# zouyuoz/SVS-UNet-PyTorch

Hardware: AMD Instinct MI355X
Metric: spectrogram-tiles/sec (512x128) U-Net fwd+bwd (L1 train step incl. Adam) (higher is better)
Workload: dtype f32; 1 GPU; train.py L1-loss step, 512x128 tiles, batch 64 per GPU; global_batch=64, parallelism=dp1, mode=train

## Files before the change

### svs_unet_pytorch_amd/csrc/gemm_wgrad.hip

```cpp
#include <stdlib.h>

#include "gemm_pipeline.h"
#include "internal.h"
#include "mfma_split.h"

struct WgradArgs {
  const float* s; long lds; int Hs, Ws, Cs;
  const float* l; long ldl; int Hl, Wl, Cl;
  int B;
  float* slab;
  long pix_per_split;
  int ws_shift, hs_shift;
  int b_shift;
};

template <int T> __device__ __forceinline__ void load_vec(const float* p, float (&f)[T]);
template <> __device__ __forceinline__ void load_vec<4>(const float* p, float (&f)[4]) {
  const f32x4 v = *(const f32x4*)p; f[0] = v[0]; f[1] = v[1]; f[2] = v[2]; f[3] = v[3];
}
template <> __device__ __forceinline__ void load_vec<2>(const float* p, float (&f)[2]) {
  const float2 v = *(const float2*)p; f[0] = v.x; f[1] = v.y;
}
template <int T> __device__ __forceinline__ void store_vec(float* p, const float (&f)[T]);
template <> __device__ __forceinline__ void store_vec<4>(float* p, const float (&f)[4]) { *(f32x4*)p = (f32x4){f[0], f[1], f[2], f[3]}; }
// ... 162 lines not shown

  auto multiply = [&](int buf) __attribute__((always_inline)) {
    if constexpr (SPLIT) {
      float ga[4][TM], gb[4][TN];
#pragma unroll
      for (int k = 0; k < 4; ++k) {
        const int kr = 4 * q + k;
        load_vec<TM>(&As[buf][kr * LDA + wm * (TM * 16) + TM * lrow], ga[k]);
        load_vec<TN>(&Bs[buf][kr * LDB + wn * (TN * 16) + TN * lrow], gb[k]);
      }
      SvsSplitA sa[TM];
      SvsSplitB sb[TN];
#pragma unroll
      for (int i = 0; i < TM; ++i) sa[i] = svs_split_a(ga[0][i], ga[1][i], ga[2][i], ga[3][i]);
#pragma unroll
      for (int j = 0; j < TN; ++j) sb[j] = svs_split_b(gb[0][j], gb[1][j], gb[2][j], gb[3][j]);
      svs_mma_split<TM, TN>(acc, sa, sb);
    } else {
#pragma unroll
    for (int k = 0; k < 4; ++k) {
      float fa[TM], fb[TN];
      const int kr = 4 * q + k;
      load_vec<TM>(&As[buf][kr * LDA + wm * (TM * 16) + TM * lrow], fa);
      load_vec<TN>(&Bs[buf][kr * LDB + wn * (TN * 16) + TN * lrow], fb);
#pragma unroll
      for (int i = 0; i < TM; ++i)
#pragma unroll
        for (int j = 0; j < TN; ++j)
          acc[i][j] = __builtin_amdgcn_mfma_f32_16x16x4f32(fa[i], fb[j], acc[i][j], 0, 0, 0);
    }
    }
  };
  auto fetch = [&](int pk, auto setc) __attribute__((always_inline)) {
    constexpr int set_ = decltype(setc)::value;
    if (SKIP) load_tile_skip(pk, ra[set_], rb[set_]);
    else load_tile(pk, ra[set_], rb[set_]);
  };
  svs_k_loop<PF>(first_valid((int)p_begin), (int)p_end, [&](int pk) { return first_valid(pk + 16); }, fetch, store_tile, multiply);

  float* slab = p.slab + (long)blockIdx.z * p.Cs * Ntot;
#pragma unroll
  for (int i = 0; i < TM; ++i)
#pragma unroll
    for (int r = 0; r < 4; ++r) {
      const int cs = cs0 + wm * (TM * 16) + TM * (4 * q + r) + i;
      const int n = n0 + wn * (TN * 16) + TN * lrow;
      if (n < Ntot) {
        float v[TN];
#pragma unroll
        for (int j = 0; j < TN; ++j) v[j] = acc[i][j][r];
        store_vec<TN>(&slab[(long)cs * Ntot + n], v);
      }
    }
}

struct WgWinArgs {
  const float* s; long lds; const float* l; long ldl;
  int B, Hs, Ws, Cs, Hl, Wl, Cl;
  float* slab;
  int ntiles, tiles_per_block;
};

template <int MT>
__global__ __launch_bounds__(256, 2) void wgrad_window_kernel(WgWinArgs p) {
  constexpr int TH = 4, TW = 16, KS = 4 / MT, CSB = 16 * MT;
  constexpr int LS = CSB + 16;
  constexpr int LH = 2 * TH + 3, LW = 2 * TW + 3, LL = 24;
  constexpr int NS = TH * TW * (CSB / 4), NL = LH * LW * 4;
  constexpr int RS = (NS + 255) / 256, RL = (NL + 255) / 256;
  constexpr int KSTEPS = TH * TW / 4 / KS;
  constexpr unsigned OOB = 0x80000000u;
  __shared__ __attribute__((aligned(16))) float Ssm[TH * TW * LS];
  __shared__ __attribute__((aligned(16))) float Lsm[LH * LW * LL];
  const int t = threadIdx.x, lane = t & 63, wave = t >> 6;
  const int lrow = lane & 15, q = lane >> 4;
  const int mt = wave % MT, half = wave / MT;
  const int mchunks = p.Cs / CSB;
  const int m0 = (blockIdx.y % mchunks) * CSB, cl0 = (blockIdx.y / mchunks) * 16;
  const int tiles_w = (p.Ws + TW - 1) / TW, tiles_h = (p.Hs + TH - 1) / TH;
  const int tile_lo = blockIdx.x * p.tiles_per_block;
  const int tile_hi = min(tile_lo + p.tiles_per_block, p.ntiles);

  f32x4 sreg[RS], lreg[RL];
  auto fetch = [&](int tile) {
    const int tw0 = (tile % tiles_w) * TW, th0 = ((tile / tiles_w) % tiles_h) * TH;
    const long b = tile / (tiles_w * tiles_h);
    const __amdgpu_buffer_rsrc_t rs = __builtin_amdgcn_make_buffer_rsrc((void*)(p.s + b * p.Hs * p.Ws * p.lds), 0, OOB, 0x00020000);
    const __amdgpu_buffer_rsrc_t rl = __builtin_amdgcn_make_buffer_rsrc((void*)(p.l + b * p.Hl * p.Wl * p.ldl), 0, OOB, 0x00020000);
#pragma unroll
    for (int r = 0; r < RS; ++r) {
      const int e = t + 256 * r;
      const int c4 = e % (CSB / 4), px = e / (CSB / 4);
      const int sh = th0 + px / TW, sw = tw0 + px % TW;
      const bool ok = e < NS && sh < p.Hs && sw < p.Ws;
      const unsigned vo = ok ? (unsigned)(((sh * p.Ws + sw) * (int)p.lds + m0 + c4 * 4) * 4) : OOB;
      sreg[r] = __builtin_bit_cast(f32x4, __builtin_amdgcn_raw_buffer_load_b128(rs, (int)vo, 0, 0));
    }
#pragma unroll
    for (int r = 0; r < RL; ++r) {
      const int e = t + 256 * r;
      const int c4 = e & 3, px = e >> 2;
      const int ih = 2 * th0 - 2 + px / LW, iw = 2 * tw0 - 2 + px % LW;
      const bool ok = e < NL && (unsigned)ih < (unsigned)p.Hl && (unsigned)iw < (unsigned)p.Wl;
      const unsigned vo = ok ? (unsigned)(((ih * p.Wl + iw) * (int)p.ldl + cl0 + c4 * 4) * 4) : OOB;
      lreg[r] = __builtin_bit_cast(f32x4, __builtin_amdgcn_raw_buffer_load_b128(rl, (int)vo, 0, 0));
    }
  };
  auto stage = [&]() {
#pragma unroll
    for (int r = 0; r < RS; ++r) {
      const int e = t + 256 * r;
      if (e < NS) *(f32x4*)(&Ssm[(e / (CSB / 4)) * LS + (e % (CSB / 4)) * 4]) = sreg[r];
    }
#pragma unroll
    for (int r = 0; r < RL; ++r) {
      const int e = t + 256 * r;
      if (e < NL) *(f32x4*)(&Lsm[(e >> 2) * LL + (e & 3) * 4]) = lreg[r];
    }
  };

  f32x4 acc[25];
#pragma unroll
  for (int i = 0; i < 25; ++i) acc[i] = (f32x4){0.f, 0.f, 0.f, 0.f};
  const float* abase = &Ssm[(half * (TH / KS) * TW + q) * LS + mt * 16 + lrow];
  const float* bbase = &Lsm[(half * (TH / KS) * 2 * LW + 2 * q) * LL + lrow];

  if (tile_lo < tile_hi) fetch(tile_lo);
  for (int tile = tile_lo; tile < tile_hi; ++tile) {
    __syncthreads();
    stage();
    __syncthreads();
    if (tile + 1 < tile_hi) fetch(tile + 1);
#pragma unroll
    for (int ks = 0; ks < KSTEPS; ++ks) {
      const int sh = ks / 4, sg = ks % 4;
      const float a = abase[(sh * TW + sg * 4) * LS];
#pragma unroll
      for (int tap = 0; tap < 25; ++tap) {
        const int kh = tap / 5, kw = tap % 5;
        const float bv = bbase[((2 * sh + kh) * LW + 8 * sg + kw) * LL];
        acc[tap] = __builtin_amdgcn_mfma_f32_16x16x4f32(a, bv, acc[tap], 0, 0, 0);
      }
    }
  }
  const int Ntot = 25 * p.Cl;
  float* slab = p.slab + ((long)blockIdx.x * KS + half) * p.Cs * Ntot;
#pragma unroll
  for (int tap = 0; tap < 25; ++tap)
#pragma unroll
    for (int r = 0; r < 4; ++r)
      slab[(long)(m0 + mt * 16 + 4 * q + r) * Ntot + tap * p.Cl + cl0 + lrow] = acc[tap][r];
}

__global__ __launch_bounds__(256) void wgrad_reduce_kernel(const float* __restrict__ slab, int ksplit, int Cs, int Cl,
                                                           float* __restrict__ dw) {
  __shared__ float tile[25][65];
  const int clt = Cl < 64 ? Cl : 64;
  const int cs = blockIdx.x, cl0 = blockIdx.y * clt;
  const long zstride = (long)Cs * Cl * 25;
  const float* src0 = slab + (long)cs * 25 * Cl + cl0;
  const int q4 = clt >> 2;
  for (int e = threadIdx.x; e < 25 * q4; e += 256) {
    const int tap = e / q4, cl = (e - tap * q4) * 4;
    const float* src = src0 + (long)tap * Cl + cl;
    f32x4 acc = {0.f, 0.f, 0.f, 0.f};
    int z = 0;
    for (; z + 4 <= ksplit; z += 4, src += 4 * zstride) {
      const f32x4 a = *(const f32x4*)src, b = *(const f32x4*)(src + zstride), c = *(const f32x4*)(src + 2 * zstride), d = *(const f32x4*)(src + 3 * zstride);
      acc += a; acc += b; acc += c; acc += d;
    }
    for (; z < ksplit; ++z, src += zstride) acc += *(const f32x4*)src;
    tile[tap][cl] = acc[0]; tile[tap][cl + 1] = acc[1]; tile[tap][cl + 2] = acc[2]; tile[tap][cl + 3] = acc[3];
  }
  __syncthreads();
  float* dst = dw + ((long)cs * Cl + cl0) * 25;
  for (int e = threadIdx.x; e < 25 * clt; e += 256) {
    const int cl = e / 25, tap = e - cl * 25;
    dst[e] = tile[tap][cl];
  }
}

struct WgradTile { int cfg, BM, BN, ksplit; long pps; };
static WgradTile plan_wgrad(int B, int Hs, int Ws, int Cs, int Cl) {
  WgradTile pl{};
  if (Cs % 128 == 0) { pl.cfg = 0; pl.BM = 128; }
  else if (Cs % 64 == 0) { pl.cfg = 1; pl.BM = 64; }
  else { pl.cfg = 2; pl.BM = 32; }
  if (pl.cfg == 0 && ((long)B * Hs * Ws <= 1024 || Cl <= 32)) { pl.cfg = 1; pl.BM = 64; }
  if (svs_tune_on(SVS_TUNE_WGRAD_CFG)) {
    const int c = (int)svs_tune(SVS_TUNE_WGRAD_CFG);
    if (c == 0 && Cs % 128 == 0) { pl.cfg = 0; pl.BM = 128; }
    if (c == 1 && Cs % 64 == 0) { pl.cfg = 1; pl.BM = 64; }
    if (c == 2 && Cs % 32 == 0) { pl.cfg = 2; pl.BM = 32; }
  }
  pl.BN = 128;
  const long P = (long)B * Hs * Ws;
  const long blocks_mn = (long)(Cs / pl.BM) * ((25L * Cl + pl.BN - 1) / pl.BN);
  long ks = (1024 + blocks_mn - 1) / blocks_mn;
  const long cap = P / 128 > 1 ? P / 128 : 1;
  if (ks > cap) ks = cap;
  if (ks > 512) ks = 512;
  if (ks < 1) ks = 1;
  if (svs_tune_on(SVS_TUNE_WGRAD_KSPLIT)) { long f = svs_tune(SVS_TUNE_WGRAD_KSPLIT); if (f >= 1 && f <= cap) ks = f; }
  long pps = (P + ks - 1) / ks;
  pps = (pps + 15) / 16 * 16;
  ks = (P + pps - 1) / pps;
  pl.ksplit = (int)ks;
  pl.pps = pps;
  return pl;
}

#define WG_GROUPS 8

struct WgWinPlan { int eligible, use, MT, gy, gx, tpb, ntiles, nslab; };
static WgWinPlan plan_wgrad_window(int B, int Hs, int Ws, int Cs, int Cl) {
  WgWinPlan w{};
  w.eligible = (Cl == 16 || Cl == 32) && (Cs == 32 || Cs == 64 || Cs == 128);
  w.ntiles = B * ((Hs + 3) / 4) * ((Ws + 15) / 16);
  w.use = w.eligible && w.ntiles >= 1024;
  if (svs_tune_on(SVS_TUNE_WGRAD_WINDOW)) { const int f = (int)svs_tune(SVS_TUNE_WGRAD_WINDOW); w.use = (f == 0) ? 0 : (f == 2) ? w.eligible : w.use; }
  if (!w.eligible) return w;
  w.MT = (Cs % 64 == 0) ? 4 : 2;
  w.gy = (Cs / (16 * w.MT)) * (Cl / 16);
  int gx = 512 / w.gy;
  if (gx > w.ntiles) gx = w.ntiles;
  w.tpb = (w.ntiles + gx - 1) / gx;
  w.gx = (w.ntiles + w.tpb - 1) / w.tpb;
  w.nslab = w.gx * (4 / w.MT);
  return w;
}

static constexpr int wgrad_gemm_pf(int BM, bool skip) { return skip && BM != 32 ? 2 : 1; }

struct WgradPlan {
  WgWinPlan win;
  WgradTile tile;
  int WM, WN;
  bool skip, split;
  dim3 grid;
  int nslab;
};
static WgradPlan plan_wgrad_call(int B, int Hs, int Ws, int Cs, int Cl, long lds, int Hl, int Wl, long ldl) {
  WgradPlan p{};
  p.win = plan_wgrad_window(B, Hs, Ws, Cs, Cl);
  p.win.use = p.win.use && (long)Hs * Ws * lds * 4 < (1L << 31) && (long)Hl * Wl * ldl * 4 < (1L << 31);
  if (p.win.use) {
    p.grid = dim3(p.win.gx, p.win.gy);
    p.nslab = p.win.nslab;
    return p;
  }
  p.tile = plan_wgrad(B, Hs, Ws, Cs, Cl);
  p.WM = p.tile.cfg == 0 ? 2 : 1;
  p.WN = 4 / p.WM;
  const bool can_skip = B >= 16 && (B & (B - 1)) == 0 && (Ws & (Ws - 1)) == 0 && (long)B * Hs * Ws * lds * 4 < (1L << 31);
  const long f = svs_tune(SVS_TUNE_WGRAD_SKIP);
  p.skip = f == 0 ? false : f == 2 ? can_skip : can_skip && Ws <= 8;
  p.split = svs_tune(SVS_TUNE_MFMA_SPLIT) > 0;
  p.grid = dim3((unsigned)(Cs / p.tile.BM), (unsigned)((25 * Cl + p.tile.BN - 1) / p.tile.BN), (unsigned)p.tile.ksplit);
  p.nslab = p.tile.ksplit;
  return p;
}

size_t svs_wgrad_gemm_workspace(int B, int Hs, int Ws, int Cs, int Cl) {
  const WgWinPlan w = plan_wgrad_window(B, Hs, Ws, Cs, Cl);
  int nslab = plan_wgrad(B, Hs, Ws, Cs, Cl).ksplit;
  if (w.eligible && w.nslab > nslab) nslab = w.nslab;
  return ((size_t)nslab + WG_GROUPS) * Cs * 25 * Cl * sizeof(float);
}

static int wgrad_reduce_run(const float* slabs, int nslab, int Cs, int Cl, float* dw, float* tmp, hipStream_t stream) {
  const long n = (long)Cs * 25 * Cl;
  if (nslab > 2 * WG_GROUPS) {
    const int per = (nslab + WG_GROUPS - 1) / WG_GROUPS;
    const int groups = (nslab + per - 1) / per;
    if (int rc = svs_reduce_slabs_run(slabs, nslab, per, groups, n, tmp, stream)) return rc;
    slabs = tmp;
    nslab = groups;
  }
  hipLaunchKernelGGL(wgrad_reduce_kernel, dim3((unsigned)Cs, (unsigned)((Cl + 63) / 64)), dim3(256), 0, stream, slabs, nslab, Cs,
                     Cl, dw);
  SVS_CHECK_LAUNCH("wgrad_reduce");
  return SVS_OK;
}

template <bool SPLIT, int BM, int WM, int WN>
static void launch_wgrad_tile(const WgradArgs& a, const WgradPlan& p, hipStream_t stream) {
  if (p.skip) hipLaunchKernelGGL((wgrad_gemm_kernel<BM, 128, WM, WN, true, SPLIT, wgrad_gemm_pf(BM, true)>), p.grid, dim3(256), 0, stream, a);
  else hipLaunchKernelGGL((wgrad_gemm_kernel<BM, 128, WM, WN, false, SPLIT, wgrad_gemm_pf(BM, false)>), p.grid, dim3(256), 0, stream, a);
}
template <bool SPLIT>
static void launch_wgrad_gemm(const WgradArgs& a, const WgradPlan& p, hipStream_t stream) {
  switch (p.tile.cfg) {
    case 0: launch_wgrad_tile<SPLIT, 128, 2, 2>(a, p, stream); break;
    case 1: launch_wgrad_tile<SPLIT, 64, 1, 4>(a, p, stream); break;
    default: launch_wgrad_tile<SPLIT, 32, 1, 4>(a, p, stream); break;
  }
}

int svs_wgrad_gemm_run(const float* s, long lds, int B, int Hs, int Ws, int Cs, const float* l, long ldl, int Hl,
                       int Wl, int Cl, float* dw, void* ws, size_t ws_bytes, hipStream_t stream, const char* who) {
  SVS_REQUIRE(s && l && dw, "%s: null pointer", who);
  SVS_REQUIRE(Cs >= 32 && Cs % 32 == 0 && Cl >= 16 && Cl % 4 == 0, "%s: unsupported channels Cs=%d Cl=%d", who, Cs, Cl);
  SVS_REQUIRE(Hs == svs_conv_out(Hl) && Ws == svs_conv_out(Wl), "%s: small grid %dx%d does not match %dx%d", who, Hs, Ws, Hl, Wl);
  SVS_REQUIRE(lds >= Cs && lds % 4 == 0 && ldl >= Cl && ldl % 4 == 0, "%s: bad ld", who);
  SVS_REQUIRE(svs_aligned16(s) && svs_aligned16(l) && svs_aligned16(ws), "%s: pointers must be 16-byte aligned", who);
  const size_t need = svs_wgrad_gemm_workspace(B, Hs, Ws, Cs, Cl);
  if (!ws || ws_bytes < need) {
    svs_set_error("%s: workspace too small (%zu < %zu)", who, ws_bytes, need);
    return SVS_ERR_WORKSPACE;
  }
  const WgradPlan p = plan_wgrad_call(B, Hs, Ws, Cs, Cl, lds, Hl, Wl, ldl);
  if (p.win.use) {
    WgWinArgs wa{s, lds, l, ldl, B, Hs, Ws, Cs, Hl, Wl, Cl, (float*)ws, p.win.ntiles, p.win.tpb};
    if (p.win.MT == 4) hipLaunchKernelGGL((wgrad_window_kernel<4>), p.grid, dim3(256), 0, stream, wa);
    else hipLaunchKernelGGL((wgrad_window_kernel<2>), p.grid, dim3(256), 0, stream, wa);
    SVS_CHECK_LAUNCH("wgrad_window");
  } else {
    WgradArgs a{};
    a.s = s; a.lds = lds; a.Hs = Hs; a.Ws = Ws; a.Cs = Cs;
    a.l = l; a.ldl = ldl; a.Hl = Hl; a.Wl = Wl; a.Cl = Cl;
    a.B = B; a.slab = (float*)ws; a.pix_per_split = p.tile.pps;
    auto log2_or_neg = [](int v) { int s = 0; while ((1 << s) < v) ++s; return (1 << s) == v ? s : -1; };
    a.ws_shift = log2_or_neg(Ws); a.hs_shift = log2_or_neg(Hs);
    SVS_REQUIRE((long)B * Hs * Ws < (1L << 31), "%s: pixel count exceeds 2^31", who);
    SVS_REQUIRE((long)B * Hl * Wl * ldl * 4 < (1L << 31) && (long)(p.tile.pps + 16) * lds * 4 < (1L << 31),
                "%s: operand views need 64-bit offsets; split the batch", who);
    if (p.skip) a.b_shift = log2_or_neg(B);
    if (p.split) launch_wgrad_gemm<true>(a, p, stream);
    else launch_wgrad_gemm<false>(a, p, stream);
    SVS_CHECK_LAUNCH("wgrad_gemm");
  }
  if (svs_tune_flag(SVS_TUNE_SKIP_REDUCE)) return SVS_OK;
  return wgrad_reduce_run((const float*)ws, p.nslab, Cs, Cl, dw, (float*)ws + (size_t)p.nslab * Cs * 25 * Cl, stream);
}

int svs_wgrad_gemm_describe(int B, int Hs, int Ws, int Cs, int Cl, char* buf, size_t n) {
  const WgradPlan p = plan_wgrad_call(B, Hs, Ws, Cs, Cl, Cs, 2 * Hs, 2 * Ws, Cl);
  if (p.win.use) snprintf(buf, n, "wgrad_window_kernel<%d>", p.win.MT);
  else snprintf(buf, n, "wgrad_gemm_kernel<%d, %d, %d, %d, %s, %s, %d>", p.tile.BM, p.tile.BN, p.WM, p.WN, p.skip ? "true" : "false",
                p.split ? "true" : "false", wgrad_gemm_pf(p.tile.BM, p.skip));
  return p.nslab;
}
```

### svs_unet_pytorch_amd/csrc/internal.h

```cpp
#pragma once
#include "common.h"

enum { SVS_MODE_GATHER = 0, SVS_MODE_PARITY = 1 };

int svs_conv_gemm_run(int mode, const float* x, long ldx, int B, int H, int W, int C, const float* wp,
                      const float* bias, const float* scale, const float* shift, float slope, float* y, long ldy,
                      int Ho, int Wo, int N, int accumulate, void* ws, size_t ws_bytes, hipStream_t stream,
                      const char* who, float* stats = nullptr, int stats_cap = 0, int* stats_nblk = nullptr);
int svs_bn_finalize_run(const void* partial, int nblk, long P, int C, float eps, float momentum, float* running_mean,
                        float* running_var, long long* nbt, float* save_mean, float* save_invstd, hipStream_t stream);
int svs_bn_fin_act_apply_run(const void* partial, int rows, const float* raw, long ldr, long P, int C, long pixels_per_sample,
                             const float* gamma, const float* beta, float eps, float momentum, float* running_mean,
                             float* running_var, long long* nbt, float* save_mean, float* save_invstd, float slope,
                             const float* drop, float* y, long ldy, hipStream_t stream);
struct SvsSumJobs { int njobs; const float* partial[12]; int nblk[12]; int C[12]; float* out[12]; };
int svs_channel_sum_finalize_multi_run(const SvsSumJobs& jobs, hipStream_t stream);
size_t svs_bn_partial_floats(long P, int C);
int svs_bn_partial_rows(long P, int C);
size_t svs_conv_gemm_workspace(int mode, int B, int H, int W, int C, int Ho, int Wo, int N);

int svs_wgrad_gemm_run(const float* s, long lds, int B, int Hs, int Ws, int Cs, const float* l, long ldl, int Hl,
                       int Wl, int Cl, float* dw, void* ws, size_t ws_bytes, hipStream_t stream, const char* who);
size_t svs_wgrad_gemm_workspace(int B, int Hs, int Ws, int Cs, int Cl);

int svs_conv_c1_run(const float* x, int B, int H, int W, const float* w, const float* bias, const float* scale,
                    const float* shift, float slope, float* y, long ldy, int N, int accumulate, hipStream_t stream,
                    const char* who, long half = 0);
int svs_deconv_to1_run(const float* x, long ldx, int B, int H, int W, int C, const float* w, const float* bias,
                       float* y, int Ho, int Wo, int apply_sigmoid, hipStream_t stream, const char* who, long half = 0);
int svs_wgrad_c1_run(const float* s, long lds, int B, int Hs, int Ws, int Cs, const float* l, int Hl, int Wl,
                     float* dw, void* ws, size_t ws_bytes, hipStream_t stream, const char* who, long half = 0);
size_t svs_wgrad_c1_workspace(int B, int Hs, int Ws, int Cs);

int svs_channel_sum_run(const float* x, long ldx, long P, int C, float* out, void* ws, size_t ws_bytes, hipStream_t stream);
int svs_sum_run(const float* x, long n, float* out, void* ws, size_t ws_bytes, hipStream_t stream);
int svs_sigmoid_bwd_run(const float* mask, const float* dmask, long n, float* d_logit, hipStream_t stream);

int svs_reduce_slabs_run(const float* slab, int nslab, int per, int groups, long n, float* out, hipStream_t stream);

struct SvsPackJob { const float* w; float* wp; int N, C, kind, first_block; };
struct SvsPackJobs { SvsPackJob j[20]; int n; };
int svs_pack_all_run(SvsPackJobs& jobs, hipStream_t stream);

int svs_bn_bwd_run(const float* dy, long lddy, const float* raw, long ldr, long P, int C, long pixels_per_sample,
                   const float* gamma, const float* beta, const float* save_mean, const float* save_invstd, float slope,
                   const float* drop, float* d_raw, float* dgamma, float* dbeta, float* dbias, void* ws, size_t ws_bytes,
                   hipStream_t stream, float* dbias_partial = nullptr, SvsSumJobs* defer = nullptr);

int svs_fft_twiddles(int n, hipStream_t stream, const float2** out);
int svs_fft_hann(int n, hipStream_t stream, const float** out);

int svs_conv_gemm_describe(int mode, int B, int H, int W, int C, int Ho, int Wo, int N, long ldx, char* buf, size_t n);
int svs_wgrad_gemm_describe(int B, int Hs, int Ws, int Cs, int Cl, char* buf, size_t n);
int svs_conv_bf16_describe(int mode, int B, int H, int W, int C, int Ho, int Wo, int N, char* buf, size_t n);
```

### svs_unet_pytorch_amd/csrc/special.hip

```cpp
#include "internal.h"

struct C1Args {
  const float* x; int B, H, W;
  const float* w;
  const float* bias; const float* scale; const float* shift; float slope;
  float* y; long ldy; int Ho, Wo; int accumulate;
  long half;
};

__device__ __forceinline__ long chan_off(long pix, long ld, int sub, int subs_per_half, long half) {
  return pix * ld + (half ? (sub >= subs_per_half ? half + (sub - subs_per_half) * 4 : sub * 4) : sub * 4);
}

template <int COUT>
__global__ __launch_bounds__(256) void conv_c1_kernel(C1Args p) {
  constexpr int G = COUT / 4;
  constexpr int LD = COUT + 4;
  __shared__ __attribute__((aligned(16))) float tile[256 * LD];
  const float* __restrict__ w = p.w;
  const long P = (long)p.B * p.Ho * p.Wo;
  const long pix0 = (long)blockIdx.x * 256;
  const long pix = pix0 + threadIdx.x;
  if (pix < P) {
    const unsigned upix = (unsigned)pix, utmp = upix / (unsigned)p.Wo;
// ... 288 lines not shown
  constexpr int G = CS / 4;
  constexpr int PL = 256 / G;
  __shared__ float red[4][25 * CS];
  const int t = threadIdx.x;
  const int cg = t % G, pl = t / G;
  const long P = (long)p.B * p.Hs * p.Ws;
  const long p0 = (long)blockIdx.x * p.pix_per_block;
  long p1 = p0 + p.pix_per_block;
  if (p1 > P) p1 = P;
  f32x4 acc[25];
#pragma unroll
  for (int k = 0; k < 25; ++k) acc[k] = (f32x4){0.f, 0.f, 0.f, 0.f};
  for (long pix = p0 + pl; pix < p1; pix += PL) {
    const int j = (int)(pix % p.Ws);
    const long tmp = pix / p.Ws;
    const int i = (int)(tmp % p.Hs);
    const long b = tmp / p.Hs;
    const f32x4 s4 = *(const f32x4*)(p.s + chan_off(pix, p.lds, cg, G / 2, p.half));
    const float* img = p.l + b * p.Hl * p.Wl;
    constexpr int NM = (25 + G - 1) / G;
    float mine[NM];
#pragma unroll
    for (int m = 0; m < NM; ++m) {
      const int tap = cg + G * m;
      const int kh = tap / 5, kw = tap - kh * 5;
      const int ih = 2 * i - 2 + kh, iw = 2 * j - 2 + kw;
      float lv = 0.f;
      if (tap < 25 && (unsigned)ih < (unsigned)p.Hl && (unsigned)iw < (unsigned)p.Wl) lv = img[(long)ih * p.Wl + iw];
      mine[m] = lv;
    }
    const int group = (t & 63) & ~(G - 1);
#pragma unroll
    for (int tap = 0; tap < 25; ++tap) {
      const float lv = __shfl(mine[tap / G], group | (tap % G), 64);
      acc[tap] += s4 * lv;
    }
  }
#pragma unroll
  for (int k = 0; k < 25; ++k)
#pragma unroll
    for (int c = 0; c < 4; ++c) {
      float v = acc[k][c];
#pragma unroll
      for (int s = G; s < 64; s <<= 1) v += __shfl_xor(v, s, 64);
      acc[k][c] = v;
    }
  const int lane = t & 63, wave = t >> 6;
  if (lane < G) {
#pragma unroll
    for (int k = 0; k < 25; ++k)
#pragma unroll
      for (int c = 0; c < 4; ++c) red[wave][(lane * 4 + c) * 25 + k] = acc[k][c];
  }
  __syncthreads();
  float* out = p.slab + (long)blockIdx.x * (25 * CS);
  for (int i = t; i < 25 * CS; i += 256) out[i] = (red[0][i] + red[1][i]) + (red[2][i] + red[3][i]);
}

template <int CS>
__global__ __launch_bounds__(256) void wgrad_c1_mfma_kernel(WgC1Args p, int ntiles, int tiles_per_wave) {
  constexpr int TH = 4, TW = 16, MT = CS / 16;
  constexpr int LS = (CS == 32) ? 48 : 16;
  constexpr int LH = 2 * TH + 3, LW = 2 * TW + 3, LWP = LW + 1;
  constexpr int NSP = TH * TW * (CS / 4) / 64;
  constexpr int NLP = (LH * LW + 63) / 64;
  __shared__ __attribute__((aligned(16))) float Ssm[4][TH * TW * LS];
  __shared__ float Lsm[4][LH * LWP];
  const int t = threadIdx.x, lane = t & 63, wave = t >> 6;
  const int lrow = lane & 15, q = lane >> 4;
  float* const sS = Ssm[wave];
  float* const sL = Lsm[wave];
  const int tiles_w = (p.Ws + TW - 1) / TW, tiles_h = (p.Hs + TH - 1) / TH;
  const int gw = blockIdx.x * 4 + wave;
  const int tile_lo = gw * tiles_per_wave;
  const int tile_hi = min(tile_lo + tiles_per_wave, ntiles);

  f32x4 sreg[NSP];
  float lreg[NLP];
  auto fetch = [&](int tile) {
    const int tw0 = (tile % tiles_w) * TW, th0 = ((tile / tiles_w) % tiles_h) * TH;
    const long b = tile / (tiles_w * tiles_h);
#pragma unroll
    for (int r = 0; r < NSP; ++r) {
      const int e = lane + 64 * r;
      const int c4 = e % (CS / 4), px = e / (CS / 4);
      const int sh = th0 + px / TW, sw = tw0 + px % TW;
      f32x4 v = {0.f, 0.f, 0.f, 0.f};
      if (sh < p.Hs && sw < p.Ws) v = *(const f32x4*)(p.s + chan_off((b * p.Hs + sh) * p.Ws + sw, p.lds, c4, CS / 8, p.half));
      sreg[r] = v;
    }
    const float* img = p.l + b * p.Hl * p.Wl;
#pragma unroll
    for (int r = 0; r < NLP; ++r) {
      const int e = lane + 64 * r;
      const int wr = e / LW, wc = e % LW;
      const int ih = 2 * th0 - 2 + wr, iw = 2 * tw0 - 2 + wc;
      float v = 0.f;
      if (e < LH * LW && (unsigned)ih < (unsigned)p.Hl && (unsigned)iw < (unsigned)p.Wl) v = img[(long)ih * p.Wl + iw];
      lreg[r] = v;
    }
  };
  auto stage = [&]() {
#pragma unroll
    for (int r = 0; r < NSP; ++r) {
      const int e = lane + 64 * r;
      *(f32x4*)(&sS[(e / (CS / 4)) * LS + (e % (CS / 4)) * 4]) = sreg[r];
    }
#pragma unroll
    for (int r = 0; r < NLP; ++r) {
      const int e = lane + 64 * r;
      if (e < LH * LW) sL[(e / LW) * LWP + e % LW] = lreg[r];
    }
  };
  f32x4 acc[MT][2];
#pragma unroll
  for (int i = 0; i < MT; ++i) { acc[i][0] = (f32x4){0.f, 0.f, 0.f, 0.f}; acc[i][1] = acc[i][0]; }
  int boff[2];
#pragma unroll
  for (int nt = 0; nt < 2; ++nt) {
    const int tap = min(nt * 16 + lrow, 24);
    boff[nt] = (tap / 5) * LWP + tap % 5 + 2 * q;
  }
  if (tile_lo < tile_hi) fetch(tile_lo);
  for (int tile = tile_lo; tile < tile_hi; ++tile) {
    stage();
    if (tile + 1 < tile_hi) fetch(tile + 1);
#pragma unroll
    for (int ks = 0; ks < TH * TW / 4; ++ks) {
      const int sh = ks / 4, sg = ks % 4;
      float bv[2];
#pragma unroll
      for (int nt = 0; nt < 2; ++nt) bv[nt] = sL[boff[nt] + 2 * sh * LWP + 8 * sg];
#pragma unroll
      for (int i = 0; i < MT; ++i) {
        const float a = sS[(sh * TW + sg * 4 + q) * LS + i * 16 + lrow];
#pragma unroll
        for (int nt = 0; nt < 2; ++nt) acc[i][nt] = __builtin_amdgcn_mfma_f32_16x16x4f32(a, bv[nt], acc[i][nt], 0, 0, 0);
      }
    }
  }
  float* out = p.slab + (long)gw * (25 * CS);
#pragma unroll
  for (int i = 0; i < MT; ++i)
#pragma unroll
    for (int nt = 0; nt < 2; ++nt) {
      const int tap = nt * 16 + lrow;
      if (tap < 25) {
#pragma unroll
        for (int r = 0; r < 4; ++r) out[(i * 16 + 4 * q + r) * 25 + tap] = acc[i][nt][r];
      }
    }
}

__global__ __launch_bounds__(256) void reduce_slabs_kernel(const float* __restrict__ slab, int nslab, int per, long n,
                                                           float* __restrict__ out) {
  const long i = ((long)blockIdx.x * 256 + threadIdx.x) * 4;
  if (i >= n) return;
  const int z0 = blockIdx.y * per;
  int z1 = z0 + per;
  if (z1 > nslab) z1 = nslab;
  const float* src = slab + (long)z0 * n + i;
  f32x4 s = {0.f, 0.f, 0.f, 0.f};
  int z = z0;
  for (; z + 4 <= z1; z += 4, src += 4 * n) {
    const f32x4 a = *(const f32x4*)src, b = *(const f32x4*)(src + n), c = *(const f32x4*)(src + 2 * n), d = *(const f32x4*)(src + 3 * n);
    s += a; s += b; s += c; s += d;
  }
  for (; z < z1; ++z, src += n) s += *(const f32x4*)src;
  *(f32x4*)(out + (long)blockIdx.y * n + i) = s;
}

int svs_reduce_slabs_run(const float* slab, int nslab, int per, int groups, long n, float* out, hipStream_t stream) {
  hipLaunchKernelGGL(reduce_slabs_kernel, dim3((unsigned)((n / 4 + 255) / 256), (unsigned)groups), dim3(256), 0, stream, slab, nslab, per, n, out);
  SVS_CHECK_LAUNCH("reduce_slabs");
  return SVS_OK;
}

#define C1_GROUPS 32

static int wgrad_c1_blocks(long P) {
  long nb = (P + 2047) / 2048;
  if (nb > 1024) nb = 1024;
  if (nb < 1) nb = 1;
  return (int)nb;
}

size_t svs_wgrad_c1_workspace(int B, int Hs, int Ws, int Cs) {
  (void)B; (void)Hs; (void)Ws;
  return (size_t)(1024 + C1_GROUPS) * 25 * Cs * sizeof(float);
}

int svs_wgrad_c1_run(const float* s, long lds, int B, int Hs, int Ws, int Cs, const float* l, int Hl, int Wl,
                     float* dw, void* ws, size_t ws_bytes, hipStream_t stream, const char* who, long half) {
  SVS_REQUIRE(s && l && dw, "%s: null pointer", who);
  SVS_REQUIRE(Cs == 16 || Cs == 32, "%s: supports Cs=16/32, got %d", who, Cs);
  SVS_REQUIRE(Hs == svs_conv_out(Hl) && Ws == svs_conv_out(Wl), "%s: grid mismatch", who);
  SVS_REQUIRE(lds >= (half ? Cs / 2 : Cs) && lds % 4 == 0 && svs_aligned16(s), "%s: bad view", who);
  const long P = (long)B * Hs * Ws;
  const int nb = wgrad_c1_blocks(P);
  const size_t need = svs_wgrad_c1_workspace(B, Hs, Ws, Cs);
  if (!ws || ws_bytes < need) {
    svs_set_error("%s: workspace too small (%zu < %zu)", who, ws_bytes, need);
    return SVS_ERR_WORKSPACE;
  }
  WgC1Args a{s, lds, B, Hs, Ws, l, Hl, Wl, (float*)ws, (P + nb - 1) / nb, half};
  int nslab = nb;
  const int ntiles = B * ((Hs + 3) / 4) * ((Ws + 15) / 16);
  if (ntiles >= 256) {
    int waves = ntiles < 1024 ? ntiles : 1024;
    waves = (waves + 3) / 4 * 4;
    if (waves > 1024) waves = 1024;
    const int tpw = (ntiles + waves - 1) / waves;
    waves = ((ntiles + tpw - 1) / tpw + 3) / 4 * 4;
    nslab = waves;
    if (Cs == 16) hipLaunchKernelGGL(wgrad_c1_mfma_kernel<16>, dim3(waves / 4), dim3(256), 0, stream, a, ntiles, tpw);
    else hipLaunchKernelGGL(wgrad_c1_mfma_kernel<32>, dim3(waves / 4), dim3(256), 0, stream, a, ntiles, tpw);
  } else if (Cs == 16) hipLaunchKernelGGL(wgrad_c1_kernel<16>, dim3(nb), dim3(256), 0, stream, a);
  else hipLaunchKernelGGL(wgrad_c1_kernel<32>, dim3(nb), dim3(256), 0, stream, a);
  SVS_CHECK_LAUNCH("wgrad_c1");
  const long n = 25L * Cs;
  float* tmp = (float*)ws + (size_t)nslab * n;
  const int groups = nslab < C1_GROUPS ? nslab : C1_GROUPS;
  const int per = (nslab + groups - 1) / groups;
  const unsigned gx = (unsigned)((n / 4 + 255) / 256);
  hipLaunchKernelGGL(reduce_slabs_kernel, dim3(gx, (unsigned)groups), dim3(256), 0, stream, (const float*)ws, nslab, per, n, tmp);
  SVS_CHECK_LAUNCH("reduce_slabs");
  hipLaunchKernelGGL(reduce_slabs_kernel, dim3(gx, 1), dim3(256), 0, stream, (const float*)tmp, groups, groups, n, dw);
  SVS_CHECK_LAUNCH("reduce_slabs");
  return SVS_OK;
}
```

Measured before the change: 20190 tiles/s.

## Fuse two-pass split-K weight-gradient reductions into single-kernel in-block group sums

Replaces the two-launch slab reduction (grouped reduce into a temp buffer, then a final reduce) with one kernel that splits slabs into groups across threads, accumulates partial sums in LDS, and sums the groups before writing dW. This applies to both the generic wgrad GEMM path and the conv1 wgrad path. Loads are issued in unrolled batches behind a scheduling barrier to raise memory-level parallelism, and the temp workspace is dropped. The split-K count for the 128-wide tile config is also lowered so all blocks fit within 512, which trades less reduction traffic for possibly lower GEMM occupancy.

```diff
diff --git a/svs_unet_pytorch_amd/csrc/gemm_wgrad.hip b/svs_unet_pytorch_amd/csrc/gemm_wgrad.hip
--- a/svs_unet_pytorch_amd/csrc/gemm_wgrad.hip
+++ b/svs_unet_pytorch_amd/csrc/gemm_wgrad.hip
@@ -338,33 +338,56 @@
       slab[(long)(m0 + mt * 16 + 4 * q + r) * Ntot + tap * p.Cl + cl0 + lrow] = acc[tap][r];
 }
 
-__global__ __launch_bounds__(256) void wgrad_reduce_kernel(const float* __restrict__ slab, int ksplit, int Cs, int Cl,
-                                                           float* __restrict__ dw) {
-  __shared__ float tile[25][65];
-  const int clt = Cl < 64 ? Cl : 64;
-  const int cs = blockIdx.x, cl0 = blockIdx.y * clt;
-  const long zstride = (long)Cs * Cl * 25;
-  const float* src0 = slab + (long)cs * 25 * Cl + cl0;
-  const int q4 = clt >> 2;
-  for (int e = threadIdx.x; e < 25 * q4; e += 256) {
-    const int tap = e / q4, cl = (e - tap * q4) * 4;
-    const float* src = src0 + (long)tap * Cl + cl;
-    f32x4 acc = {0.f, 0.f, 0.f, 0.f};
-    int z = 0;
-    for (; z + 4 <= ksplit; z += 4, src += 4 * zstride) {
-      const f32x4 a = *(const f32x4*)src, b = *(const f32x4*)(src + zstride), c = *(const f32x4*)(src + 2 * zstride), d = *(const f32x4*)(src + 3 * zstride);
-      acc += a; acc += b; acc += c; acc += d;
-    }
-    for (; z < ksplit; ++z, src += zstride) acc += *(const f32x4*)src;
-    tile[tap][cl] = acc[0]; tile[tap][cl + 1] = acc[1]; tile[tap][cl + 2] = acc[2]; tile[tap][cl + 3] = acc[3];
+#define WG_GROUPS 8
+#define WGSUM_LDS 1632
+
+struct WgSumArgs { const float* slab; float* dw; int nslab, per, groups, Cs, Cl, clt, tpt; };
+__device__ __forceinline__ int small_div(int n, float rcp_d) { return (int)(((float)n + 0.5f) * rcp_d); }
+template <int U, bool ONE>
+__global__ __launch_bounds__(256) void wgrad_sum_kernel(WgSumArgs p) {
+  __shared__ float part[WGSUM_LDS];
+  const int ncl = (p.Cl + p.clt - 1) / p.clt, groups = ONE ? 1 : p.groups;
+  const int cs = blockIdx.x, cl0 = (ONE ? blockIdx.y : blockIdx.y % ncl) * p.clt, t0 = ONE ? 0 : (blockIdx.y / ncl) * p.tpt;
+  const int cln = p.Cl - cl0 < p.clt ? p.Cl - cl0 : p.clt, tn = ONE ? 25 : 25 - t0 < p.tpt ? 25 - t0 : p.tpt;
+  const int q4 = cln >> 2, E = tn * q4, ldp = cln + 1;
+  const float rE = __builtin_amdgcn_rcpf((float)E), rq4 = __builtin_amdgcn_rcpf((float)q4), rtn = __builtin_amdgcn_rcpf((float)tn);
+  const long zs = (long)p.Cs * 25 * p.Cl;
+  for (int t = threadIdx.x; t < E * groups; t += blockDim.x) {
+    const int g = ONE ? 0 : small_div(t, rE), e = t - g * E, tap = small_div(e, rq4), cl = (e - tap * q4) * 4;
+    const int z0 = g * p.per, z1 = z0 + p.per < p.nslab ? z0 + p.per : p.nslab;
+    const float* src = p.slab + (long)z0 * zs + ((long)cs * 25 + t0 + tap) * p.Cl + cl0 + cl;
+    f32x4 acc = {0.f, 0.f, 0.f, 0.f}, v[U];
+    int z = z0;
+    for (; z + U <= z1; z += U, src += U * zs) {
+#pragma unroll
+      for (int k = 0; k < U; ++k) v[k] = *(const f32x4*)(src + k * zs);
+      __builtin_amdgcn_sched_barrier(0);
+#pragma unroll
+      for (int k = 0; k < U; ++k) acc += v[k];
+    }
+    if (U > 1 && z < z1) {
+      const int r = z1 - z;
+#pragma unroll
+      for (int k = 0; k < U; ++k) v[k] = *(const f32x4*)(src + (k < r ? k : r - 1) * zs);
+      __builtin_amdgcn_sched_barrier(0);
+#pragma unroll
+      for (int k = 0; k < U; ++k) acc = k < r ? acc + v[k] : acc;
+    }
+    float* d = part + (g * tn + tap) * ldp + cl;
+    d[0] = acc[0]; d[1] = acc[1]; d[2] = acc[2]; d[3] = acc[3];
   }
   __syncthreads();
-  float* dst = dw + ((long)cs * Cl + cl0) * 25;
-  for (int e = threadIdx.x; e < 25 * clt; e += 256) {
-    const int cl = e / 25, tap = e - cl * 25;
-    dst[e] = tile[tap][cl];
-  }
-}
+  float* dst = p.dw + ((long)cs * p.Cl + cl0) * 25 + t0;
+  for (int i = threadIdx.x; i < cln * tn; i += blockDim.x) {
+    const int cl = ONE ? i / 25 : small_div(i, rtn), tap = i - cl * tn;
+    float s = 0.f;
+    for (int g = 0; g < groups; ++g) s += part[(g * tn + tap) * ldp + cl];
+    dst[cl * 25 + tap] = s;
+  }
+}
+
+struct WgradSplit { long blocks; bool within; };
+static constexpr WgradSplit wgrad_split(int cfg) { return cfg == 0 ? WgradSplit{512, true} : WgradSplit{1024, false}; }
 
 struct WgradTile { int cfg, BM, BN, ksplit; long pps; };
 static WgradTile plan_wgrad(int B, int Hs, int Ws, int Cs, int Cl) {
@@ -382,7 +405,8 @@
   pl.BN = 128;
   const long P = (long)B * Hs * Ws;
   const long blocks_mn = (long)(Cs / pl.BM) * ((25L * Cl + pl.BN - 1) / pl.BN);
-  long ks = (1024 + blocks_mn - 1) / blocks_mn;
+  const WgradSplit sp = wgrad_split(pl.cfg);
+  long ks = sp.within ? sp.blocks / blocks_mn : (sp.blocks + blocks_mn - 1) / blocks_mn;
   const long cap = P / 128 > 1 ? P / 128 : 1;
   if (ks > cap) ks = cap;
   if (ks > 512) ks = 512;
@@ -395,8 +419,6 @@
   pl.pps = pps;
   return pl;
 }
-
-#define WG_GROUPS 8
 
 struct WgWinPlan { int eligible, use, MT, gy, gx, tpb, ntiles, nslab; };
 static WgWinPlan plan_wgrad_window(int B, int Hs, int Ws, int Cs, int Cl) {
@@ -451,22 +473,38 @@
   const WgWinPlan w = plan_wgrad_window(B, Hs, Ws, Cs, Cl);
   int nslab = plan_wgrad(B, Hs, Ws, Cs, Cl).ksplit;
   if (w.eligible && w.nslab > nslab) nslab = w.nslab;
-  return ((size_t)nslab + WG_GROUPS) * Cs * 25 * Cl * sizeof(float);
-}
-
-static int wgrad_reduce_run(const float* slabs, int nslab, int Cs, int Cl, float* dw, float* tmp, hipStream_t stream) {
-  const long n = (long)Cs * 25 * Cl;
+  return (size_t)nslab * Cs * 25 * Cl * sizeof(float);
+}
+
+static int wgrad_sum_run(const float* slabs, int nslab, int Cs, int Cl, float* dw, hipStream_t stream) {
+  WgSumArgs a{slabs, dw, nslab, nslab, 1, Cs, Cl, Cl < 64 ? Cl : 64, 25};
   if (nslab > 2 * WG_GROUPS) {
-    const int per = (nslab + WG_GROUPS - 1) / WG_GROUPS;
-    const int groups = (nslab + per - 1) / per;
-    if (int rc = svs_reduce_slabs_run(slabs, nslab, per, groups, n, tmp, stream)) return rc;
-    slabs = tmp;
-    nslab = groups;
-  }
-  hipLaunchKernelGGL(wgrad_reduce_kernel, dim3((unsigned)Cs, (unsigned)((Cl + 63) / 64)), dim3(256), 0, stream, slabs, nslab, Cs,
-                     Cl, dw);
-  SVS_CHECK_LAUNCH("wgrad_reduce");
+    a.per = (nslab + WG_GROUPS - 1) / WG_GROUPS;
+    a.groups = (nslab + a.per - 1) / a.per;
+  }
+  const int ncl = (Cl + a.clt - 1) / a.clt, rows = a.groups * (a.clt / 4);
+  int nchunk = 1, threads = 256;
+  if (a.groups > 1) {
+    for (int tasks = 256; ; tasks >>= 1) {
+      const int t = tasks / rows < 1 ? 1 : tasks / rows > 25 ? 25 : tasks / rows;
+      nchunk = (25 + t - 1) / t;
+      a.tpt = (25 + nchunk - 1) / nchunk;
+      if ((long)Cs * ncl * nchunk >= 512 || tasks == 64) break;
+    }
+    threads = (rows * a.tpt + 63) / 64 * 64;
+  }
+  SVS_REQUIRE(threads <= 256 && a.groups * a.tpt * (a.clt + 1) <= WGSUM_LDS, "wgrad_sum: tile of %d x %d x %d does not fit", a.groups, a.tpt, a.clt);
+  const dim3 grid((unsigned)Cs, (unsigned)(ncl * nchunk));
+  const dim3 block(threads);
+  if (a.groups > 1) hipLaunchKernelGGL((wgrad_sum_kernel<4, false>), grid, block, 0, stream, a);
+  else if (a.per > 1) hipLaunchKernelGGL((wgrad_sum_kernel<4, true>), grid, block, 0, stream, a);
+  else hipLaunchKernelGGL((wgrad_sum_kernel<1, true>), grid, block, 0, stream, a);
+  SVS_CHECK_LAUNCH("wgrad_sum");
   return SVS_OK;
+}
+extern "C" int svs_wgrad_sum_test(const float* slabs, int nslab, int Cs, int Cl, float* dw, hipStream_t stream) {
+  SVS_REQUIRE(slabs && dw && nslab >= 1 && Cs >= 1 && Cl >= 16 && Cl % 4 == 0, "svs_wgrad_sum_test: bad arguments");
+  return wgrad_sum_run(slabs, nslab, Cs, Cl, dw, stream);
 }
 
 template <bool SPLIT, int BM, int WM, int WN>
@@ -517,7 +555,7 @@
     SVS_CHECK_LAUNCH("wgrad_gemm");
   }
   if (svs_tune_flag(SVS_TUNE_SKIP_REDUCE)) return SVS_OK;
-  return wgrad_reduce_run((const float*)ws, p.nslab, Cs, Cl, dw, (float*)ws + (size_t)p.nslab * Cs * 25 * Cl, stream);
+  return wgrad_sum_run((const float*)ws, p.nslab, Cs, Cl, dw, stream);
 }
 
 int svs_wgrad_gemm_describe(int B, int Hs, int Ws, int Cs, int Cl, char* buf, size_t n) {
diff --git a/svs_unet_pytorch_amd/csrc/internal.h b/svs_unet_pytorch_amd/csrc/internal.h
--- a/svs_unet_pytorch_amd/csrc/internal.h
+++ b/svs_unet_pytorch_amd/csrc/internal.h
@@ -36,7 +36,8 @@
 int svs_sum_run(const float* x, long n, float* out, void* ws, size_t ws_bytes, hipStream_t stream);
 int svs_sigmoid_bwd_run(const float* mask, const float* dmask, long n, float* d_logit, hipStream_t stream);
 
-int svs_reduce_slabs_run(const float* slab, int nslab, int per, int groups, long n, float* out, hipStream_t stream);
+extern "C" int svs_wgrad_sum_test(const float* slabs, int nslab, int Cs, int Cl, float* dw, hipStream_t stream);
+extern "C" int svs_reduce_slabs_test(const float* slabs, int nslab, long n, float* out, hipStream_t stream);
 
 struct SvsPackJob { const float* w; float* wp; int N, C, kind, first_block; };
 struct SvsPackJobs { SvsPackJob j[20]; int n; };
diff --git a/svs_unet_pytorch_amd/csrc/special.hip b/svs_unet_pytorch_amd/csrc/special.hip
--- a/svs_unet_pytorch_amd/csrc/special.hip
+++ b/svs_unet_pytorch_amd/csrc/special.hip
@@ -464,31 +464,55 @@
     }
 }
 
-__global__ __launch_bounds__(256) void reduce_slabs_kernel(const float* __restrict__ slab, int nslab, int per, long n,
-                                                           float* __restrict__ out) {
-  const long i = ((long)blockIdx.x * 256 + threadIdx.x) * 4;
-  if (i >= n) return;
-  const int z0 = blockIdx.y * per;
-  int z1 = z0 + per;
-  if (z1 > nslab) z1 = nslab;
-  const float* src = slab + (long)z0 * n + i;
-  f32x4 s = {0.f, 0.f, 0.f, 0.f};
-  int z = z0;
-  for (; z + 4 <= z1; z += 4, src += 4 * n) {
-    const f32x4 a = *(const f32x4*)src, b = *(const f32x4*)(src + n), c = *(const f32x4*)(src + 2 * n), d = *(const f32x4*)(src + 3 * n);
-    s += a; s += b; s += c; s += d;
-  }
-  for (; z < z1; ++z, src += n) s += *(const f32x4*)src;
-  *(f32x4*)(out + (long)blockIdx.y * n + i) = s;
-}
-
-int svs_reduce_slabs_run(const float* slab, int nslab, int per, int groups, long n, float* out, hipStream_t stream) {
-  hipLaunchKernelGGL(reduce_slabs_kernel, dim3((unsigned)((n / 4 + 255) / 256), (unsigned)groups), dim3(256), 0, stream, slab, nslab, per, n, out);
+#define C1_GROUPS 32
+
+__global__ __launch_bounds__(4 * C1_GROUPS) void reduce_slabs_kernel(const float* __restrict__ slab, int nslab, int per, int groups,
+                                                                     long n, float* __restrict__ out) {
+  constexpr int U = 16;
+  __shared__ f32x4 part[C1_GROUPS][4];
+  const int g = threadIdx.x >> 2, c = threadIdx.x & 3;
+  const long i = ((long)blockIdx.x * 4 + c) * 4;
+  f32x4 s = {0.f, 0.f, 0.f, 0.f}, v[U];
+  const int z0 = g * per, z1 = z0 + per < nslab ? z0 + per : nslab;
+  if (i < n && z0 < z1) {
+    const float* src = slab + (long)z0 * n + i;
+    int z = z0;
+    for (; z + U <= z1; z += U, src += U * n) {
+#pragma unroll
+      for (int k = 0; k < U; ++k) v[k] = *(const f32x4*)(src + k * n);
+      __builtin_amdgcn_sched_barrier(0);
+#pragma unroll
+      for (int k = 0; k < U; ++k) s += v[k];
+    }
+    if (z < z1) {
+      const int r = z1 - z;
+#pragma unroll
+      for (int k = 0; k < U; ++k) v[k] = *(const f32x4*)(src + (k < r ? k : r - 1) * n);
+      __builtin_amdgcn_sched_barrier(0);
+#pragma unroll
+      for (int k = 0; k < U; ++k) s = k < r ? s + v[k] : s;
+    }
+  }
+  part[g][c] = s;
+  __syncthreads();
+  if (g == 0 && i < n) {
+    f32x4 t = {0.f, 0.f, 0.f, 0.f};
+    for (int h = 0; h < groups; ++h) t += part[h][c];
+    *(f32x4*)(out + i) = t;
+  }
+}
+
+static int reduce_slabs_run(const float* slab, int nslab, long n, float* out, hipStream_t stream) {
+  const int groups = nslab < C1_GROUPS ? nslab : C1_GROUPS;
+  const int per = (nslab + groups - 1) / groups;
+  hipLaunchKernelGGL(reduce_slabs_kernel, dim3((unsigned)((n / 4 + 3) / 4)), dim3(4 * groups), 0, stream, slab, nslab, per, groups, n, out);
   SVS_CHECK_LAUNCH("reduce_slabs");
   return SVS_OK;
 }
-
-#define C1_GROUPS 32
+extern "C" int svs_reduce_slabs_test(const float* slabs, int nslab, long n, float* out, hipStream_t stream) {
+  SVS_REQUIRE(slabs && out && nslab >= 1 && n >= 4 && n % 4 == 0, "svs_reduce_slabs_test: bad arguments");
+  return reduce_slabs_run(slabs, nslab, n, out, stream);
+}
 
 static int wgrad_c1_blocks(long P) {
   long nb = (P + 2047) / 2048;
@@ -499,7 +523,7 @@
 
 size_t svs_wgrad_c1_workspace(int B, int Hs, int Ws, int Cs) {
   (void)B; (void)Hs; (void)Ws;
-  return (size_t)(1024 + C1_GROUPS) * 25 * Cs * sizeof(float);
+  return (size_t)1024 * 25 * Cs * sizeof(float);
 }
 
 int svs_wgrad_c1_run(const float* s, long lds, int B, int Hs, int Ws, int Cs, const float* l, int Hl, int Wl,
@@ -530,14 +554,5 @@
   } else if (Cs == 16) hipLaunchKernelGGL(wgrad_c1_kernel<16>, dim3(nb), dim3(256), 0, stream, a);
   else hipLaunchKernelGGL(wgrad_c1_kernel<32>, dim3(nb), dim3(256), 0, stream, a);
   SVS_CHECK_LAUNCH("wgrad_c1");
-  const long n = 25L * Cs;
-  float* tmp = (float*)ws + (size_t)nslab * n;
-  const int groups = nslab < C1_GROUPS ? nslab : C1_GROUPS;
-  const int per = (nslab + groups - 1) / groups;
-  const unsigned gx = (unsigned)((n / 4 + 255) / 256);
-  hipLaunchKernelGGL(reduce_slabs_kernel, dim3(gx, (unsigned)groups), dim3(256), 0, stream, (const float*)ws, nslab, per, n, tmp);
-  SVS_CHECK_LAUNCH("reduce_slabs");
-  hipLaunchKernelGGL(reduce_slabs_kernel, dim3(gx, 1), dim3(256), 0, stream, (const float*)tmp, groups, groups, n, dw);
-  SVS_CHECK_LAUNCH("reduce_slabs");
-  return SVS_OK;
-}
+  return reduce_slabs_run((const float*)ws, nslab, 25L * Cs, dw, stream);
+}
```

New measurement: 20340 tiles/s (median of 6 runs). No clear change (+0.7%).
